# autonomousvision/sdfstudio

Measured on NVIDIA H100. Metric: rays/sec at 4096 rays x 128 samples, higher is better.
Workload: dtype bf16x3 (fp32 accumulate)

## Files before the change

include/sdfb200_debug.h:

```cpp
#ifndef SDFB200_DEBUG_H_
#define SDFB200_DEBUG_H_
#include "sdfb200.h"
#ifdef __cplusplus
extern "C" {
#endif

int sdfb200_debug_tc_gemm(const float* A, const float* W, int32_t K, int32_t N, int32_t mode_ts, int32_t planes, float* D,
                          void* scratch, void* stream);

int sdfb200_debug_tc_linear(int32_t planes, int32_t epi, const float* X, int32_t ldx, const float* W, const float* bias, float* Y,
                            int32_t ldy, int64_t M, int32_t Np, int32_t Kp, const float* aux, int32_t ldaux, int32_t aux_cols,
                            void* scratch, void* stream);

int sdfb200_debug_tc_timing(long long* host_out_512);

#ifdef __cplusplus
}
#endif
#endif
```

sdfstudio_b200/csrc/field_tc.h:

```cpp
#pragma once
#include "field_plan.h"

namespace sdfb200 {


constexpr int kEpiWarps = 8;
constexpr int kEpiThreads = kEpiWarps * 32;
constexpr int kTcThreads = kEpiThreads + 128;
constexpr int kEncThreads = 96;
constexpr int kEncItems0 = 288, kEncItems1 = 256, kEncItems2 = 224;
static_assert(kEncItems0 + kEncItems1 + kEncItems2 == 768, "the encoder warps' items cover the tile");
__host__ __device__ constexpr int enc_item_begin(int w) { return w == 0 ? 0 : w == 1 ? kEncItems0 : w == 2 ? kEncItems0 + kEncItems1 : 768; }
constexpr int kConsumerRegs = 216;
constexpr int kProducerRegs = 72;
static_assert(2 * (kConsumerRegs - 168) <= 168 - kProducerRegs, "setmaxnreg.inc would wait for registers nobody frees");
constexpr int kStages = 5;
constexpr int kKB = 16;
constexpr int kMaxGridDim = 32;
constexpr int kMaxPe = 60;
constexpr int kPeRows = 64;
constexpr int kInK = 96;
constexpr float kHalfPiF = 1.5707963267948966f;
constexpr uint32_t kAPlane = 32 * 2048;
constexpr uint32_t kImgPlane = (kInK / 8) * 128 * 16;
__host__ __device__ constexpr uint32_t tc_stage_bytes(int planes) { return (uint32_t)planes * 256 * kKB * 2; }

enum { PRM_B_G0 = 0, PRM_B_G1, PRM_W_G2 , PRM_B_C0, PRM_B_C1, PRM_W_C2 , kPrmRows = PRM_W_C2 + 3 };
enum { HS_SDF = 0, HS_GRAD , HS_RGB = HS_GRAD + 3 , kHsRows = HS_RGB + 3 };

struct TcSmem { size_t a, ring, prm, hs, coldesc, hx, bytes; };
__host__ __device__ constexpr TcSmem tc_smem(int planes) {
  TcSmem s{};
  s.ring = s.a + (size_t)planes * kAPlane;
  s.prm = s.ring + (size_t)kStages * tc_stage_bytes(planes);
  s.hs = s.prm + kPrmRows * 256 * 4;
  s.coldesc = s.hs + 2 * kHsRows * 128 * 4;
  s.hx = s.coldesc + 96 * 16;
  s.bytes = s.hx + 128 * 8;
  return s;
}
constexpr size_t kSmemPerBlock = 232448;
constexpr size_t kStaticSmem = 1024;
static_assert(tc_smem(2).bytes + kStaticSmem <= kSmemPerBlock, "shared memory of k_field_tc at two planes");

constexpr size_t kFragWords = 64 * 256;
struct TcScratch { size_t sig, h2, slots, slot_bytes, geo, cs, jpe, jg, bytes; };
__host__ __device__ constexpr TcScratch tc_scratch(int planes) {
  TcScratch s{};
  s.h2 = s.sig + kFragWords * 4;
  s.slots = s.h2 + (size_t)planes * kFragWords * 4;
  s.cs = s.geo + (size_t)planes * kImgPlane;
  s.jpe = s.cs + (size_t)planes * kImgPlane;
  s.jg = s.jpe + (size_t)kPeRows * 128 * 4;
  s.slot_bytes = s.jg + (size_t)kMaxGridDim * 3 * 128 * 4;
  s.bytes = s.slots + 2 * s.slot_bytes;
  return s;
}
__host__ __device__ constexpr size_t kScratchPerCta(int planes) { return tc_scratch(planes).bytes; }

__host__ __device__ constexpr int tc_layer_np(int L) { return L == L_B0 ? 128 : 256; }
__host__ __device__ constexpr int tc_layer_k(int L) { return L == L_G0 || L == L_C0MISC ? kInK : 256; }
__host__ __device__ constexpr int tc_layer_kblk(int L) { return kKB * 256 / tc_layer_np(L); }
__host__ __device__ constexpr int tc_layer_nkb(int L) { return tc_layer_k(L) / tc_layer_kblk(L); }
constexpr bool tc_blocks_fill_stages() {
  for (int L = 0; L < L_COUNT; ++L)
    if (tc_layer_np(L) * tc_layer_kblk(L) != 256 * kKB || tc_layer_kblk(L) % 16 != 0 || tc_layer_k(L) % tc_layer_kblk(L) != 0) return false;
  return true;
}
static_assert(tc_blocks_fill_stages(), "every streamed weight block must be one full ring stage of whole K steps");

struct TcLayer {
  unsigned long long w_off;
};

struct TcArgs {
  sdfb200_grid_t grid;
  TcLayer layer[L_COUNT];
  int use_grid, pe_degree, use_pe, contraction, pe_dim, grid_dim, app_dim, use_n_dot_v;
  int mode;
  int n_samples, has_bins, n_tiles;
  long long n_points;
  float rgb_padding, cos_anneal;
  const float *origins, *directions, *bins, *appearance, *variance, *beta, *beta_min;
  const void* table;
  const char* blob;
  unsigned long long b_g0, b_g1, b_g2, w_g2, b_c0, b_c1, w_c2, b_c2;
  char* scratch;
  sdfb200_field_out_t out;
  int render;
  sdfb200_field_render_t rnd;
};

int launch_field_tc_p2_torch(const TcArgs& a, int grid, size_t smem, cudaStream_t st);
int launch_field_tc_p2_tcnn(const TcArgs& a, int grid, size_t smem, cudaStream_t st);
int launch_field_tc_p1_torch(const TcArgs& a, int grid, size_t smem, cudaStream_t st);
int launch_field_tc_p1_tcnn(const TcArgs& a, int grid, size_t smem, cudaStream_t st);

}
```

sdfstudio_b200/csrc/field_tc_kernel.cuh:

```cuda
#pragma once
#include "field_tc.h"
#include "grid.cuh"
#include "tc_common.cuh"

namespace sdfb200 {
using namespace tc;

__device__ __forceinline__ void named_sync(int id, int n) { asm volatile("bar.sync %0, %1;" ::"r"(id), "r"(n) : "memory"); }
constexpr int kEncBar = 3;

struct PointGeom { float px, py, pz, dx, dy, dz, delta, t0, t1; long long ray; };
__device__ __forceinline__ PointGeom point_geom(const TcArgs& a, long long p) {
  PointGeom g;
  g.dx = g.dy = g.dz = 0.f; g.delta = 0.f; g.t0 = g.t1 = 0.f;
  g.ray = a.has_bins ? p / a.n_samples : p;
  if (a.has_bins) {
    const int smp = (int)(p - g.ray * a.n_samples);
    const float t0 = __ldg(a.bins + g.ray * (a.n_samples + 1) + smp);
    g.t0 = t0;
    g.t1 = __ldg(a.bins + g.ray * (a.n_samples + 1) + smp + 1);
    g.delta = __fsub_rn(g.t1, t0);
    g.dx = __ldg(a.directions + g.ray * 3); g.dy = __ldg(a.directions + g.ray * 3 + 1); g.dz = __ldg(a.directions + g.ray * 3 + 2);
    g.px = __fadd_rn(__ldg(a.origins + g.ray * 3 + 0), __fmul_rn(g.dx, t0));
    g.py = __fadd_rn(__ldg(a.origins + g.ray * 3 + 1), __fmul_rn(g.dy, t0));
    g.pz = __fadd_rn(__ldg(a.origins + g.ray * 3 + 2), __fmul_rn(g.dz, t0));
  } else {
    g.px = __ldg(a.origins + p * 3); g.py = __ldg(a.origins + p * 3 + 1); g.pz = __ldg(a.origins + p * 3 + 2);
    if (a.directions) { g.dx = __ldg(a.directions + p * 3); g.dy = __ldg(a.directions + p * 3 + 1); g.dz = __ldg(a.directions + p * 3 + 2); }
  }
  if (a.contraction != SDFB200_CONTRACT_NONE) {
    const float mag = a.contraction == SDFB200_CONTRACT_LINF
                          ? fmaxf(fabsf(g.px), fmaxf(fabsf(g.py), fabsf(g.pz)))
                          : sqrtf(__fadd_rn(__fadd_rn(__fmul_rn(g.px, g.px), __fmul_rn(g.py, g.py)), __fmul_rn(g.pz, g.pz)));
    if (mag >= 1.f) {
      const float k = __fsub_rn(2.f, __fdiv_rn(1.f, mag));
      g.px = __fmul_rn(k, __fdiv_rn(g.px, mag)); g.py = __fmul_rn(k, __fdiv_rn(g.py, mag)); g.pz = __fmul_rn(k, __fdiv_rn(g.pz, mag));
    }
  }
  return g;
}

static __device__ __forceinline__ void sincos_call(float x, float* s, float* c) { sincosf(x, s, c); }
static __device__ __forceinline__ float sin_call(float x) { return sinf(x); }

template <int P, int LAYOUT>
__device__ __forceinline__ void encode_tile_grid(const TcArgs& a, int tile, int row, int grp, uint8_t* img, uint32_t plane, float* Jg,
                                                 uint64_t pol_table) {
  const long long p_raw = (long long)tile * 128 + row;
  const long long p = p_raw < a.n_points ? p_raw : a.n_points - 1;
  const PointGeom g = point_geom(a, p);
  const float x01 = (g.px + 2.0f) * 0.25f, y01 = (g.py + 2.0f) * 0.25f, z01 = (g.pz + 2.0f) * 0.25f;
#pragma unroll 1
  for (int l = 4 * grp; l < 4 * grp + 4; ++l) {
    float o[2] = {0.f, 0.f};
    float dj[2][3] = {{0.f, 0.f, 0.f}, {0.f, 0.f, 0.f}};
    if (a.use_grid && l < a.grid.n_levels && l < a.grid.active_levels) {
      LevelCtx c;
      float tv[8][2];
      level_prepare<LAYOUT>(a.grid, l, x01, y01, z01, c);
      if (a.grid.table_dtype == SDFB200_DT_F16) level_fetch<__half, 2, true>(a.table, c, tv, pol_table);
      else level_fetch<float, 2, true>(a.table, c, tv, pol_table);
      level_finish<2, LAYOUT>(a.grid, c, tv, o, dj);
    }
    store_a<P>(img, plane, row, 2 * l, o[0]);
    store_a<P>(img, plane, row, 2 * l + 1, o[1]);
    if (a.mode != 0 && l < a.grid.n_levels) {
#pragma unroll
      for (int f = 0; f < 2; ++f) {
        const int cg = l * 2 + f;
        Jg[(cg * 3 + 0) * 128 + row] = 0.25f * dj[f][0];
        Jg[(cg * 3 + 1) * 128 + row] = 0.25f * dj[f][1];
        Jg[(cg * 3 + 2) * 128 + row] = 0.25f * dj[f][2];
      }
    }
  }
}

template <int P>
__device__ __forceinline__ void encode_tile_pe(const TcArgs& a, int tile, int row, uint8_t* img, uint32_t plane, float* Jpe) {
  const long long p_raw = (long long)tile * 128 + row;
  const long long p = p_raw < a.n_points ? p_raw : a.n_points - 1;
  const PointGeom g = point_geom(a, p);
  if (p_raw < a.n_points) {
    if (a.out.points_norm) a.out.points_norm[p] = sqrtf(__fadd_rn(__fadd_rn(__fmul_rn(g.px, g.px), __fmul_rn(g.py, g.py)), __fmul_rn(g.pz, g.pz)));
    if (a.out.points) { a.out.points[p * 3] = g.px; a.out.points[p * 3 + 1] = g.py; a.out.points[p * 3 + 2] = g.pz; }
  }
  const int deg = a.pe_degree, half = 3 * deg;
  const float pc[3] = {g.px, g.py, g.pz};
  const uint4 z4 = make_uint4(0u, 0u, 0u, 0u);
#pragma unroll 1
  for (int ch = 4; ch < kInK / 8; ++ch) store_a_chunk<P>(img, plane, row, ch, z4, z4);
#pragma unroll 1
  for (int i = 0; i < a.pe_dim; ++i) {
    const int ia = i >= half ? i - half : i;
    const int b = ia / deg, k = ia - b * deg;
    const float fr = (float)(1 << k);
    const float xb = b == 0 ? pc[0] : (b == 1 ? pc[1] : pc[2]);
    const float arg = i >= half ? xb * fr + kHalfPiF : xb * fr;
    float sv, cv;
    sincos_call(arg, &sv, &cv);
    store_a<P>(img, plane, row, 32 + i, a.use_pe ? sv : 0.f);
    if (a.mode != 0) Jpe[i * 128 + row] = a.use_pe ? fr * cv : 0.f;
  }
  store_a<P>(img, plane, row, 32 + a.pe_dim + 0, pc[0]);
  store_a<P>(img, plane, row, 32 + a.pe_dim + 1, pc[1]);
  store_a<P>(img, plane, row, 32 + a.pe_dim + 2, pc[2]);
}

template <int P>
__device__ __forceinline__ void colour_static_tile(const TcArgs& a, int tile, int row, uint8_t* img, uint32_t plane) {
  const long long p_raw = (long long)tile * 128 + row;
  const long long p = p_raw < a.n_points ? p_raw : a.n_points - 1;
  const PointGeom g = point_geom(a, p);
  const uint4 z4 = make_uint4(0u, 0u, 0u, 0u);
#pragma unroll 1
  for (int ch = 1; ch < kInK / 8; ++ch) store_a_chunk<P>(img, plane, row, ch, z4, z4);
  store_a<P>(img, plane, row, 8 + 0, g.px); store_a<P>(img, plane, row, 8 + 1, g.py); store_a<P>(img, plane, row, 8 + 2, g.pz);
#pragma unroll 1
  for (int i = 0; i < 12; ++i) {
    const int b = i >> 2;
    const float db = b == 0 ? g.dx : (b == 1 ? g.dy : g.dz);
    const float arg = db * (float)(1 << (i & 3));
    store_a<P>(img, plane, row, 8 + 3 + i, sin_call(arg));
    store_a<P>(img, plane, row, 8 + 15 + i, sin_call(arg + kHalfPiF));
  }
  store_a<P>(img, plane, row, 8 + 27, g.dx); store_a<P>(img, plane, row, 8 + 28, g.dy); store_a<P>(img, plane, row, 8 + 29, g.dz);
  if (a.appearance != nullptr) {
#pragma unroll 1
    for (int j = 0; j < a.app_dim; ++j) store_a<P>(img, plane, row, 8 + 30 + j, __ldg(a.appearance + g.ray * a.app_dim + j));
  }
}

template <int P>
struct Slot {
  uint8_t* base;
  __device__ __forceinline__ Slot(char* slots, uint32_t s) : base(reinterpret_cast<uint8_t*>(slots) + s * tc_scratch(P).slot_bytes) {}
  __device__ __forceinline__ uint8_t* geo() const { return base + tc_scratch(P).geo; }
  __device__ __forceinline__ uint8_t* cs() const { return base + tc_scratch(P).cs; }
  __device__ __forceinline__ float* jpe() const { return reinterpret_cast<float*>(base + tc_scratch(P).jpe); }
  __device__ __forceinline__ float* jg() const { return reinterpret_cast<float*>(base + tc_scratch(P).jg); }
};

#ifdef SDFB200_TC_TIMING
__device__ long long g_tc_timing[16 * 32];
#define TC_PUT(tno, k, v)                                                                                            \
  do {                                                                                                               \
    if (blockIdx.x == 0 && (tno) >= 0 && (tno) < 16) g_tc_timing[(tno) * 32 + (k)] = (v);                            \
  } while (0)
#else
#define TC_PUT(tno, k, v) do { (void)(v); } while (0)
#endif
#define TC_STAMP(k) do { if (tid == 0) TC_PUT(tile_no, k, TC_CLOCK()); } while (0)

struct TcBars {
  Handoff<kStages> ring;
  Handoff<2> enc;
  Handoff<1> a;
  Handoff<2> hs;
};

template <int P>
__device__ __forceinline__ void produce_all(const TcArgs& a, int nlayers, uint8_t* abuf, uint8_t* ring, char* slots, TcBars& b) {
  uint32_t j = 0;
  int tile_no = 0;
  for (int tile = blockIdx.x; tile < a.n_tiles; tile += gridDim.x, ++tile_no) {
    long long waited = 0;
    b.a.wait_empty(tile_no);
    b.enc.wait_full(tile_no);
    const uint8_t* geo = Slot<P>(slots, b.enc.slot(tile_no)).geo();
    mbar_arrive_expect_tx(b.a.full_bar(tile_no), (uint32_t)P * kImgPlane);
#pragma unroll
    for (int pl = 0; pl < P; ++pl) bulk_g2s(abuf + pl * kAPlane, geo + pl * kImgPlane, kImgPlane, b.a.full_bar(tile_no));
    for (int L = 0; L < nlayers; ++L) {
      for (int kb = 0; kb < tc_layer_nkb(L); ++kb, ++j)
        ring_fill(b.ring, ring, j, reinterpret_cast<const uint8_t*>(a.blob) + a.layer[L].w_off, kb, tc_stage_bytes(P), &waited);
    }
    TC_PUT(tile_no, 10, waited);
  }
}

template <int P, int L>
__device__ __forceinline__ void layer_mma(float (&acc)[4][32], bool zero, uint32_t a_base, const uint8_t* ring, Handoff<kStages>& rb, uint32_t& it,
                                          int lane, long long& waited) {
  constexpr int N = tc_layer_np(L);
  constexpr int KSTEPS = tc_layer_kblk(L) / 16;
  constexpr uint32_t lbo_b = N * 16, plane_b = N * KSTEPS * 16 * 2;
  float (&d)[N / 2] = *reinterpret_cast<float (*)[N / 2]>(&acc[0][0]);
  if (zero) {
#pragma unroll
    for (int i = 0; i < N / 2; ++i) d[i] = 0.f;
  }
#pragma unroll 1
  for (int kb = 0; kb < tc_layer_nkb(L); ++kb, ++it) {
    rb.wait_full(it, &waited);
    const uint32_t wbase = smem_u32(ring + (size_t)rb.slot(it) * tc_stage_bytes(P));
    wg_fence_acc(d);
    wg_arrive();
#pragma unroll
    for (int j = 0; j < KSTEPS; ++j) {
      const int kstep = kb * KSTEPS + j;
      wgmma_kstep_wide_ss<P, N>(d, a_desc(a_base, kstep), a_desc(a_base + kAPlane, kstep), wbase + j * 2 * lbo_b, plane_b, lbo_b);
    }
    wg_commit();
    wg_wait<0>();
    wg_fence_acc(d);
    __syncwarp();
    if (lane == 0) rb.arrive_empty(it);
  }
}

struct TileCtx {
  const TcArgs& a;
  int tid, t, wg, wrow0;
  int r0, cq;
  uint8_t* abuf;
  const float (*prm)[256];
  float (*hs)[128];
  const float4* coldesc;
  float sdf_bias;
  uint32_t* sig_s;
  uint32_t* gf_s;
  char* slots;
  __device__ __forceinline__ int unit(int c, int i) const { return (c * 16 + (i >> 1)) * kEpiThreads + tid; }
};

__device__ __forceinline__ uint32_t unorm16x2_encode(float s0, float s1) {
  const float f0 = __fadd_rn(__fmul_rn(s0, 65535.0f), 12582912.0f), f1 = __fadd_rn(__fmul_rn(s1, 65535.0f), 12582912.0f);
  return __byte_perm(__float_as_uint(f0), __float_as_uint(f1), 0x5410);
}
__device__ __forceinline__ float unorm16_lo(uint32_t w) { return __fsub_rn(__uint_as_float(__byte_perm(w, 0x4B00u, 0x5410)), 8388608.0f) * (1.0f / 65535.0f); }
__device__ __forceinline__ float unorm16_hi(uint32_t w) { return __fsub_rn(__uint_as_float(__byte_perm(w, 0x4B00u, 0x5432)), 8388608.0f) * (1.0f / 65535.0f); }

__device__ __forceinline__ void acc_shift(float (&acc)[4][32]) {
#pragma unroll
  for (int c = 0; c < 3; ++c) {
#pragma unroll
    for (int i = 0; i < 32; ++i) acc[c][i] = acc[c + 1][i];
  }
}

template <int N>
__device__ __forceinline__ void load_prm_block(const float* prow, int cq, int c, int j0, float2 (&v)[N]) {
#pragma unroll
  for (int j = 0; j < N; ++j) v[j] = *reinterpret_cast<const float2*>(prow + frag_col(cq, c, 4 * (j0 + j)));
}

template <int P>
__device__ __forceinline__ void epi_e0(const TileCtx& x, float (&acc)[4][32]) {
  const float* p_bg0 = x.prm[PRM_B_G0];
#pragma unroll 1
  for (int c = 0; c < 4; ++c, acc_shift(acc)) {
    float2 bias[8];
    load_prm_block(p_bg0, x.cq, c, 0, bias);
#pragma unroll
    for (int i = 0; i < 32; i += 2) {
      const int col = frag_col(x.cq, c, i), row = frag_row(x.r0, i);
      const float2 b2 = bias[i >> 2];
      float h0, h1, s0, s1;
      softplus100_fast(acc[0][i] + b2.x, h0, s0);
      softplus100_fast(acc[0][i + 1] + b2.y, h1, s1);
      store_a_pair<P>(x.abuf, kAPlane, row, col, h0, h1);
      if (x.a.mode != 0) x.sig_s[x.unit(c, i)] = unorm16x2_encode(s0, s1);
    }
  }
}

template <int P>
__device__ __forceinline__ void epi_e1(const TileCtx& x, int tile, float (&acc)[4][32]) {
  const TcArgs& a = x.a;
  const float* p_bg1 = x.prm[PRM_B_G1];
  const float* p_wg2 = x.prm[PRM_W_G2];
  float sp0 = 0.f, sp1 = 0.f;
#pragma unroll 1
  for (int c = 0; c < 4; ++c, acc_shift(acc)) {
    float2 bias[2], wrow[2];
#pragma unroll
    for (int i = 0; i < 32; i += 2) {
      if (i % 8 == 0) { load_prm_block(p_bg1, x.cq, c, i >> 2, bias); load_prm_block(p_wg2, x.cq, c, i >> 2, wrow); }
      const int col = frag_col(x.cq, c, i), row = frag_row(x.r0, i);
      const float2 b2 = bias[(i >> 2) & 1];
      const float2 w2 = wrow[(i >> 2) & 1];
      float h0, h1, s0, s1;
      softplus100_fast(acc[0][i] + b2.x, h0, s0);
      softplus100_fast(acc[0][i + 1] + b2.y, h1, s1);
      float& sp = frag_half(i) ? sp1 : sp0;
      sp = fmaf(w2.x, h0, sp);
      sp = fmaf(w2.y, h1, sp);
      if (a.mode != 0) {
        uint32_t hi, lo;
        split2(h0, h1, hi, lo);
        const int u = x.unit(c, i);
        x.gf_s[u] = hi;
        if (P > 1) x.gf_s[kFragWords + u] = lo;
        store_a_pair<P>(x.abuf, kAPlane, row, col, w2.x * s0, w2.y * s1);
      }
    }
  }
  sp0 = quad_sum(sp0);
  sp1 = quad_sum(sp1);
  if ((x.t & 3) < 2) {
    const int h = x.t & 1, row = x.r0 + 8 * h;
    const float sdf = (h ? sp1 : sp0) + x.sdf_bias;
    const long long p = (long long)tile * 128 + row;
    if (p < a.n_points && a.out.sdf) a.out.sdf[p] = sdf;
    if (a.mode != 0) x.hs[HS_SDF][row] = sdf;
  }
}

template <int P>
__device__ __forceinline__ void epi_eb1(const TileCtx& x, float (&acc)[4][32]) {
  uint32_t sw[16], sw_next[16];
#pragma unroll
  for (int k = 0; k < 16; ++k) sw[k] = x.sig_s[x.unit(0, 2 * k)];
#pragma unroll 1
  for (int c = 0; c < 4; ++c, acc_shift(acc)) {
    if (c < 3) {
#pragma unroll
      for (int k = 0; k < 16; ++k) sw_next[k] = x.sig_s[x.unit(c + 1, 2 * k)];
    }
#pragma unroll
    for (int i = 0; i < 32; i += 2) {
      const int col = frag_col(x.cq, c, i), row = frag_row(x.r0, i);
      const uint32_t w = sw[i >> 1];
      store_a_pair<P>(x.abuf, kAPlane, row, col, acc[0][i] * unorm16_lo(w), acc[0][i + 1] * unorm16_hi(w));
    }
    if (c < 3) {
#pragma unroll
      for (int k = 0; k < 16; ++k) sw[k] = sw_next[k];
    }
  }
}

__device__ __forceinline__ float4 col_desc(const TcArgs& a, int ip) {
  const int deg = a.pe_degree, half = 3 * deg;
  int jrow = -1, ax = -1;
  if (ip < a.pe_dim) {
    const int ia = ip >= half ? ip - half : ip;
    ax = ia < deg ? 0 : (ia < 2 * deg ? 1 : 2);
    jrow = ip * 128;
  } else if (ip - a.pe_dim < 3) {
    ax = ip - a.pe_dim;
  }
  return make_float4(__int_as_float(jrow), ax == 0 ? 1.f : 0.f, ax == 1 ? 1.f : 0.f, ax == 2 ? 1.f : 0.f);
}

template <int P>
__device__ __forceinline__ void epi_eb0(const TileCtx& x, int tile, const Slot<P>& s, const float (&acc)[4][32]) {
  const TcArgs& a = x.a;
  const float* Jpe = s.jpe();
  const float* Jg = s.jg();
  constexpr int kUnits = 11 * 64 * P, kPer = (kUnits + 127) / 128;
  uint4 v[kPer];
#pragma unroll
  for (int j = 0; j < kPer; ++j) {
    const int k = x.t + 128 * j, pl = k / (11 * 64), ch = 1 + (k - pl * 11 * 64) / 64, row = x.wrow0 + (k & 63);
    if (k < kUnits) v[j] = *reinterpret_cast<const uint4*>(s.cs() + pl * kImgPlane + ch * kAChunk + row * 16);
  }
  float g0x = 0.f, g0y = 0.f, g0z = 0.f, g1x = 0.f, g1y = 0.f, g1z = 0.f;
#pragma unroll
  for (int c = 0; c < 2; ++c) {
#pragma unroll
    for (int i = 0; i < 32; ++i) {
      const int col = frag_col(x.cq, c, i), row = frag_row(x.r0, i);
      const bool h = frag_half(i);
      float& gx = h ? g1x : g0x;
      float& gy = h ? g1y : g0y;
      float& gz = h ? g1z : g0z;
      const float g = acc[c][i];
      if (c == 0 && i < 16) {
        const bool live = col < a.grid_dim;
        const float* j = Jg + col * 3 * 128 + row;
        const float jx = live ? j[0] : 0.f, jy = live ? j[128] : 0.f, jz = live ? j[256] : 0.f;
        gx = fmaf(g, jx, gx); gy = fmaf(g, jy, gy); gz = fmaf(g, jz, gz);
      } else {
        const float4 d = x.coldesc[col - 32];
        const int jrow = __float_as_int(d.x);
        const float tv = __fmul_rn(g, jrow >= 0 ? Jpe[jrow + row] : 1.f);
        gx = fmaf(tv, d.y, gx); gy = fmaf(tv, d.z, gy); gz = fmaf(tv, d.w, gz);
      }
    }
  }
  g0x = quad_sum(g0x); g0y = quad_sum(g0y); g0z = quad_sum(g0z);
  g1x = quad_sum(g1x); g1y = quad_sum(g1y); g1z = quad_sum(g1z);
  if ((x.t & 3) < 2) {
    const int h = x.t & 1, row = x.r0 + 8 * h;
    const long long p_raw = (long long)tile * 128 + row;
    const PointGeom pg = point_geom(a, p_raw < a.n_points ? p_raw : a.n_points - 1);
    const float grx = h ? g1x : g0x, gry = h ? g1y : g0y, grz = h ? g1z : g0z;
    const float3 n = normalize_eps(grx, gry, grz);
    const float c0v[8] = {grx, gry, grz, a.use_n_dot_v ? n.x * pg.dx + n.y * pg.dy + n.z * pg.dz : 0.f, 0.f, 0.f, 0.f, 0.f};
    store_a_chunk<P>(x.abuf, kAPlane, row, 0, c0v);
    x.hs[HS_GRAD][row] = grx; x.hs[HS_GRAD + 1][row] = gry; x.hs[HS_GRAD + 2][row] = grz;
  }
#pragma unroll
  for (int j = 0; j < kPer; ++j) {
    const int k = x.t + 128 * j, pl = k / (11 * 64), ch = 1 + (k - pl * 11 * 64) / 64, row = x.wrow0 + (k & 63);
    if (k < kUnits) *reinterpret_cast<uint4*>(x.abuf + pl * kAPlane + ch * kAChunk + row * 16) = v[j];
  }
}

template <int P>
__device__ __forceinline__ void reload_h2(const TileCtx& x) {
#pragma unroll 1
  for (int c = 0; c < 4; ++c) {
#pragma unroll
    for (int i = 0; i < 32; i += 2) {
      const int col = frag_col(x.cq, c, i), row = frag_row(x.r0, i);
      const int u = x.unit(c, i);
      store_a_pair<P>(x.abuf, kAPlane, row, col, x.gf_s[u], x.gf_s[kFragWords + u]);
    }
  }
}

template <int P>
__device__ __forceinline__ void epi_ec0(const TileCtx& x, float (&acc)[4][32]) {
  const float* p_bc0 = x.prm[PRM_B_C0];
#pragma unroll 1
  for (int c = 0; c < 4; ++c, acc_shift(acc)) {
    float2 bias[8];
    load_prm_block(p_bc0, x.cq, c, 0, bias);
#pragma unroll
    for (int i = 0; i < 32; i += 2) {
      const int col = frag_col(x.cq, c, i), row = frag_row(x.r0, i);
      const float2 b2 = bias[i >> 2];
      store_a_pair<P>(x.abuf, kAPlane, row, col, fmaxf(acc[0][i] + b2.x, 0.f), fmaxf(acc[0][i + 1] + b2.y, 0.f));
    }
  }
}

__device__ __forceinline__ void epi_ec1(const TileCtx& x, float (&acc)[4][32]) {
  const float* p_bc1 = x.prm[PRM_B_C1];
  const float (*p_wc2)[256] = x.prm + PRM_W_C2;
  float r0r = 0.f, r0g = 0.f, r0b = 0.f, r1r = 0.f, r1g = 0.f, r1b = 0.f;
#pragma unroll 1
  for (int c = 0; c < 4; ++c, acc_shift(acc)) {
#pragma unroll
    for (int i = 0; i < 32; ++i) {
      const int col = frag_col(x.cq, c, i);
      const bool h = frag_half(i);
      float& rr = h ? r1r : r0r;
      float& rg = h ? r1g : r0g;
      float& rb = h ? r1b : r0b;
      const float v = fmaxf(acc[0][i] + p_bc1[col], 0.f);
      rr = fmaf(p_wc2[0][col], v, rr);
      rg = fmaf(p_wc2[1][col], v, rg);
      rb = fmaf(p_wc2[2][col], v, rb);
    }
  }
  r0r = quad_sum(r0r); r0g = quad_sum(r0g); r0b = quad_sum(r0b);
  r1r = quad_sum(r1r); r1g = quad_sum(r1g); r1b = quad_sum(r1b);
  if ((x.t & 3) < 2) {
    const int h = x.t & 1, row = x.r0 + 8 * h;
    x.hs[HS_RGB][row] = h ? r1r : r0r; x.hs[HS_RGB + 1][row] = h ? r1g : r0g; x.hs[HS_RGB + 2][row] = h ? r1b : r0b;
  }
}

struct HeadsXfer { double wtot[2][4]; float csum[2][4][8]; };
static_assert(sizeof(TcBars) + sizeof(HeadsXfer) <= kStaticSmem, "static shared memory of k_field_tc (kStaticSmem)");
enum { HR_ALPHA = HS_SDF , HR_NORMAL = HS_GRAD , HR_RGB = HS_RGB  };
struct RayEnd { int q; double tot; float last[3]; };
struct HeadsClock { long long rows, scan, sums; };

__device__ __forceinline__ float sample_mid(const TcArgs& a, long long p) {
// ... 134 lines not shown
#pragma unroll
      for (int k = 0; k < 8; ++k) s[k] += csum[w2][k];
    }
    finish_ray(ray, s[0], {s[1], s[2], s[3]}, {s[4], s[5], s[6]}, s[7], a.rnd.bg_mode, a.rnd.bg, end.last, a.rnd.clamp01, a.rnd.out.rgb,
               a.rnd.out.accumulation, a.rnd.out.normal, a.rnd.out.depth);
    const bool dens = a.rnd.from_density != 0;
    if (a.rnd.bg_transmittance) a.rnd.bg_transmittance[ray] = dens ? expf(-(float)end.tot) : (float)end.tot;
  }
  clk.sums += TC_CLOCK() - tc0;
}

__device__ __forceinline__ void heads_of(const TcArgs& a, int tile, int tile_no, int et, TcBars& b, float (*hs)[128], double* hx, HeadsXfer& xf,
                                         float& dmin, float& dmax) {
  const int ew = et >> 5, lane = et & 31;
  long long waited = 0, bar_waited = 0;
  b.hs.wait_full(tile_no, &waited);
  const long long t0 = TC_CLOCK();
  float (*h)[128] = hs + b.hs.slot(tile_no) * kHsRows;
  double* wtot = xf.wtot[tile_no & 1];
  float (*csum)[8] = xf.csum[tile_no & 1];
  HeadsClock clk{0, 0, 0};
#pragma unroll 1
  for (int q = ew; q < 4; q += kEncThreads / 32) heads_rows(a, h, hx, wtot, tile, q, lane, dmin, dmax, clk);
  if (a.render && a.n_samples > 32) {
    long long c = TC_CLOCK();
    named_sync(kEncBar, kEncThreads);
    bar_waited += TC_CLOCK() - c;
    RayEnd end{-1, 0.0, {0.f, 0.f, 0.f}};
#pragma unroll 1
    for (int q = ew; q < 4; q += kEncThreads / 32) composite_chunk(a, h, hx, wtot, csum, tile, q, lane, end, clk);
    c = TC_CLOCK();
    named_sync(kEncBar, kEncThreads);
    bar_waited += TC_CLOCK() - c;
    finish_rays(a, csum, tile, lane, end, clk);
  }
  b.hs.arrive_empty(tile_no);
  if (lane == 0) TC_PUT(tile_no, ew == 0 ? 14 : 25 + ew, TC_CLOCK() - t0);
  if (et == 0) { TC_PUT(tile_no, 17, waited); TC_PUT(tile_no, 28, clk.rows); TC_PUT(tile_no, 29, clk.scan); TC_PUT(tile_no, 30, clk.sums); TC_PUT(tile_no, 31, bar_waited); }
}

template <int P, int LAYOUT>
__device__ __forceinline__ void encode_all(const TcArgs& a, int et, char* slots, TcBars& b, uint64_t pol_table, float (*hs)[128], double* hx,
                                           HeadsXfer& xf) {
  const bool heads = a.mode != 0;
  const int ew = et >> 5, lane = et & 31;
  const int i_begin = heads ? enc_item_begin(ew) + lane : et, i_end = heads ? enc_item_begin(ew + 1) : 640, i_step = heads ? 32 : kEncThreads;
  float dmin = INFINITY, dmax = -INFINITY;
  int tile_no = 0;
  for (int tile = blockIdx.x; tile < a.n_tiles; tile += gridDim.x, ++tile_no) {
    long long waited = 0;
    b.enc.wait_empty(tile_no, &waited);
    const long long t0 = TC_CLOCK();
    const Slot<P> s(slots, b.enc.slot(tile_no));
#pragma unroll 1
    for (int i = i_begin; i < i_end; i += i_step) {
      const int row = i & 127;
      if (i < 512) encode_tile_grid<P, LAYOUT>(a, tile, row, i >> 7, s.geo(), kImgPlane, s.jg(), pol_table);
      else if (i < 640) encode_tile_pe<P>(a, tile, row, s.geo(), kImgPlane, s.jpe());
      else colour_static_tile<P>(a, tile, row, s.cs(), kImgPlane);
    }
    fence_async_global();
    b.enc.arrive_full(tile_no);
    if (et == 0) { TC_PUT(tile_no, 12, TC_CLOCK() - t0); TC_PUT(tile_no, 13, waited); }
    else if (lane == 0) TC_PUT(tile_no, 23 + ew, TC_CLOCK() - t0);
    if (heads && tile_no > 0) heads_of(a, tile - (int)gridDim.x, tile_no - 1, et, b, hs, hx, xf, dmin, dmax);
  }
  if (heads && tile_no > 0) heads_of(a, blockIdx.x + (tile_no - 1) * (int)gridDim.x, tile_no - 1, et, b, hs, hx, xf, dmin, dmax);
  if (heads && a.render && a.rnd.out.steps_minmax) {
#pragma unroll
    for (int d = 1; d < 32; d <<= 1) {
      dmin = fminf(dmin, __shfl_xor_sync(0xffffffffu, dmin, d));
      dmax = fmaxf(dmax, __shfl_xor_sync(0xffffffffu, dmax, d));
    }
    if (lane == 0 && dmin <= dmax) { atomic_min_float(a.rnd.out.steps_minmax, dmin); atomic_max_float(a.rnd.out.steps_minmax + 1, dmax); }
  }
}

template <int P, int LAYOUT>
__global__ void __launch_bounds__(kTcThreads, 1) k_field_tc(const __grid_constant__ TcArgs a) {
  extern __shared__ __align__(1024) uint8_t smem[];
  constexpr TcSmem sm = tc_smem(P);
  constexpr TcScratch scr = tc_scratch(P);
  uint8_t* abuf = smem + sm.a;
  uint8_t* ring = smem + sm.ring;
  float (*prm)[256] = reinterpret_cast<float (*)[256]>(smem + sm.prm);
  float (*hs)[128] = reinterpret_cast<float (*)[128]>(smem + sm.hs);
  float4* coldesc = reinterpret_cast<float4*>(smem + sm.coldesc);
  double* hx = reinterpret_cast<double*>(smem + sm.hx);
  __shared__ TcBars bars;
  __shared__ HeadsXfer hxf;

  const int tid = threadIdx.x, warp = tid >> 5, lane = tid & 31;
  const int nlayers = a.mode == 0 ? 2 : L_COUNT;
  char* cta_scr = a.scratch + (size_t)blockIdx.x * scr.bytes;
  char* slots = cta_scr + scr.slots;
  if (tid == 0) {
    bars.ring.init(1, kEpiWarps);
    bars.enc.init(kEncThreads, kEpiThreads);
    bars.hs.init(kEpiThreads, kEncThreads);
    bars.a.init(1, 2);
    fence_barrier_init();
  }
  {
    const char* blob = a.blob;
    const float* src[kPrmRows] = {reinterpret_cast<const float*>(blob + a.b_g0), reinterpret_cast<const float*>(blob + a.b_g1),
                                  reinterpret_cast<const float*>(blob + a.w_g2), reinterpret_cast<const float*>(blob + a.b_c0),
                                  reinterpret_cast<const float*>(blob + a.b_c1), reinterpret_cast<const float*>(blob + a.w_c2),
                                  reinterpret_cast<const float*>(blob + a.w_c2) + 256, reinterpret_cast<const float*>(blob + a.w_c2) + 512};
    for (int i = tid; i < kPrmRows * 256; i += kTcThreads) prm[i >> 8][i & 255] = src[i >> 8][i & 255];
    if (tid < 96) coldesc[tid] = col_desc(a, tid);
  }
  __syncthreads();

  if (tid >= kEpiThreads) {
    setmaxnreg_dec<kProducerRegs>();
    if (tid == kEpiThreads) produce_all<P>(a, nlayers, abuf, ring, slots, bars);
    else if (tid >= kTcThreads - kEncThreads) encode_all<P, LAYOUT>(a, tid - (kTcThreads - kEncThreads), slots, bars, l2_policy_evict_last(), hs, hx, hxf);
    return;
  }
  setmaxnreg_inc<kConsumerRegs>();

  const int wg = warp >> 2, t = tid & 127;
  const int wrow0 = wg * 64;
  const int wg_bar = 1 + wg;
  const uint32_t a_base = smem_u32(abuf) + wrow0 * 16;
  const float sdf_bias = __ldg(reinterpret_cast<const float*>(a.blob + a.b_g2));
  TileCtx x{a, tid, t, wg, wrow0, frag_row0(wrow0, t), frag_cq(t), abuf, prm, hs, coldesc, sdf_bias,
            reinterpret_cast<uint32_t*>(cta_scr + scr.sig), reinterpret_cast<uint32_t*>(cta_scr + scr.h2), slots};
  uint32_t it = 0;
  long long waited = 0;
  float acc[4][32];
#define SYNC_A()                \
  do {                          \
    fence_async_smem();         \
    named_sync(wg_bar, 128);    \
  } while (0)
#define LAYER(L, zero)                                                                                 \
  do {                                                                                                 \
    layer_mma<P, L>(acc, zero, a_base, ring, bars.ring, it, lane, waited);                             \
    named_sync(wg_bar, 128);   \
    TC_STAMP(1 + (L));                                                                                 \
  } while (0)

  int tile_no = -1;
  for (int tile = blockIdx.x; tile < a.n_tiles; tile += gridDim.x) {
    ++tile_no;
    TC_STAMP(0);
    waited = 0;
    const Slot<P> s(slots, bars.enc.slot(tile_no));
    x.hs = hs + bars.hs.slot(tile_no) * kHsRows;
    bars.a.wait_full(tile_no);
    if (a.mode == 0) bars.enc.arrive_empty(tile_no);
    TC_STAMP(8);
    LAYER(L_G0, true);
    epi_e0<P>(x, acc);
    TC_STAMP(18);
    SYNC_A();
    LAYER(L_G1, true);
    if (a.mode == 0) {
      if (t == 0) bars.a.arrive_empty(tile_no);
      epi_e1<P>(x, tile, acc);
      continue;
    }
    {
      long long hs_waited = 0;
      bars.hs.wait_empty(tile_no, &hs_waited);
      if (tid == 0) TC_PUT(tile_no, 16, hs_waited);
    }
    epi_e1<P>(x, tile, acc);
    TC_STAMP(19);
    SYNC_A();
    LAYER(L_B1, true);
    epi_eb1<P>(x, acc);
    TC_STAMP(20);
    SYNC_A();
    LAYER(L_B0, true);
    bars.enc.wait_full(tile_no);
    epi_eb0<P>(x, tile, s, acc);
    bars.enc.arrive_empty(tile_no);
    TC_STAMP(21);
    SYNC_A();
    LAYER(L_C0MISC, true);
    reload_h2<P>(x);
    TC_STAMP(22);
    SYNC_A();
    LAYER(L_C0H, false);
    epi_ec0<P>(x, acc);
    TC_STAMP(23);
    SYNC_A();
    LAYER(L_C1, true);
    if (t == 0) bars.a.arrive_empty(tile_no);
    epi_ec1(x, acc);
    bars.hs.arrive_full(tile_no);
    TC_STAMP(15);
    if (tid == 0) TC_PUT(tile_no, 9, waited);
  }
#undef SYNC_A
#undef LAYER
}

template <int P, int LAYOUT>
static int launch_field_tc(const TcArgs& a, int grid, size_t smem, cudaStream_t st) {
  SDFB_CUDA(cudaFuncSetAttribute(k_field_tc<P, LAYOUT>, cudaFuncAttributeMaxDynamicSharedMemorySize, (int)smem));
  k_field_tc<P, LAYOUT><<<grid, kTcThreads, smem, st>>>(a);
  SDFB_LAUNCHED("k_field_tc");
  return 0;
}

}
```

sdfstudio_b200/csrc/field_tc_p2_torch.cu:

```cuda
#include "field_tc_kernel.cuh"

namespace sdfb200 {
int launch_field_tc_p2_torch(const TcArgs& a, int grid, size_t smem, cudaStream_t st) { return launch_field_tc<2, SDFB200_GRID_TORCH>(a, grid, smem, st); }
}

#ifdef SDFB200_TC_TIMING
extern "C" int sdfb200_debug_tc_timing(long long* host_out_512) {
  SDFB_CUDA(cudaMemcpyFromSymbol(host_out_512, sdfb200::g_tc_timing, sizeof(long long) * 512));
  return 0;
}
#endif
```

sdfstudio_b200/csrc/grid.cuh:

```cuda
#pragma once
#include "common.cuh"

namespace sdfb200 {

constexpr uint32_t kPrimeY = 2654435761u;
constexpr uint32_t kPrimeZ = 805459861u;

__device__ __forceinline__ uint64_t l2_policy_evict_last() {
  uint64_t p;
  asm volatile("createpolicy.fractional.L2::evict_last.b64 %0, 1.0;" : "=l"(p));
  return p;
}

template <typename T, int F, bool HINT = false>
__device__ __forceinline__ void load_row(const void* table, uint64_t row, float (&v)[F], uint64_t pol = 0) {
  const T* p = reinterpret_cast<const T*>(table) + row * F;
  if constexpr (HINT) {
    static_assert(F == 2, "hinted loads are only used by the F=2 fused kernel");
    if constexpr (sizeof(T) == 4) {
      asm volatile("ld.global.nc.L2::cache_hint.v2.f32 {%0, %1}, [%2], %3;" : "=f"(v[0]), "=f"(v[1]) : "l"(p), "l"(pol));
    } else {
      uint32_t raw;
      asm volatile("ld.global.nc.L2::cache_hint.b32 %0, [%1], %2;" : "=r"(raw) : "l"(p), "l"(pol));
      const float2 t = __half22float2(*reinterpret_cast<const __half2*>(&raw));
// ... 47 lines not shown
  uint32_t idx[8];
  uint64_t base;
  float w[3], dw[3], d2w[3], s;
};

template <int LAYOUT = -1>
__device__ __forceinline__ void level_prepare(const sdfb200_grid_t& g, int l, float x, float y, float z, LevelCtx& c) {
  if constexpr (LAYOUT < 0) {
    if (g.layout == SDFB200_GRID_TORCH) level_prepare<SDFB200_GRID_TORCH>(g, l, x, y, z, c);
    else level_prepare<SDFB200_GRID_TCNN>(g, l, x, y, z, c);
    return;
  }
  constexpr bool torch = LAYOUT == SDFB200_GRID_TORCH;
  const float s = g.scale[l];
  const float xs[3] = {x, y, z};
  uint32_t lo[3], hi[3];
  c.s = s;
  c.base = g.offset[l];
#pragma unroll
  for (int d = 0; d < 3; ++d) {
    const float p = torch ? __fmul_rn(xs[d], s) : fmaf(xs[d], s, 0.5f);
    const float fl = floorf(p);
    lo[d] = (uint32_t)(int)fl;
    hi[d] = torch ? (uint32_t)(int)ceilf(p) : lo[d] + 1u;
    const float t = __fsub_rn(p, fl);
    if (g.smoothstep) {
      c.w[d] = __fmul_rn(__fmul_rn(t, t), __fsub_rn(3.0f, __fmul_rn(2.0f, t)));
      c.dw[d] = 6.f * t * (1.f - t);
      c.d2w[d] = (6.f - 12.f * t) * s * s;
    } else {
      c.w[d] = t; c.dw[d] = 1.f; c.d2w[d] = 0.f;
    }
  }
  const uint32_t mask = (1u << g.log2_hashmap_size) - 1u;
#pragma unroll
  for (int k = 0; k < 8; ++k) {
    const uint32_t ix = (k & 1) ? hi[0] : lo[0], iy = (k & 2) ? hi[1] : lo[1], iz = (k & 4) ? hi[2] : lo[2];
    const uint32_t h = ix ^ (iy * kPrimeY) ^ (iz * kPrimeZ);
    if (torch) {
      c.idx[k] = h & mask;
    } else {
      const uint32_t res = g.resolution[l];
      c.idx[k] = (g.hashed[l] ? h : ix + iy * res + iz * res * res) % g.size[l];
    }
  }
}

template <typename T, int F, bool HINT = false>
__device__ __forceinline__ void level_fetch(const void* table, const LevelCtx& c, float (&v)[8][F], uint64_t pol = 0) {
#pragma unroll
  for (int k = 0; k < 8; ++k) load_row<T, F, HINT>(table, c.base + c.idx[k], v[k], pol);
}

template <int F, int LAYOUT = -1>
__device__ __forceinline__ void level_finish(const sdfb200_grid_t& g, const LevelCtx& c, const float (&v)[8][F], float (&out)[F], float (&dout)[F][3]) {
  if (torch_layout<LAYOUT>(g)) {
    const float(&f0)[F] = v[7], (&f1)[F] = v[5], (&f2)[F] = v[4], (&f3)[F] = v[6], (&f4)[F] = v[3], (&f5)[F] = v[1], (&f6)[F] = v[0], (&f7)[F] = v[2];
    const float ox = c.w[0], oy = c.w[1], oz = c.w[2];
    const float nx = __fsub_rn(1.f, ox), ny = __fsub_rn(1.f, oy), nz = __fsub_rn(1.f, oz);
#pragma unroll
    for (int f = 0; f < F; ++f) {
      const float f03 = __fadd_rn(__fmul_rn(f0[f], ox), __fmul_rn(f3[f], nx));
      const float f12 = __fadd_rn(__fmul_rn(f1[f], ox), __fmul_rn(f2[f], nx));
      const float f56 = __fadd_rn(__fmul_rn(f5[f], ox), __fmul_rn(f6[f], nx));
      const float f47 = __fadd_rn(__fmul_rn(f4[f], ox), __fmul_rn(f7[f], nx));
      const float f0312 = __fadd_rn(__fmul_rn(f03, oy), __fmul_rn(f12, ny));
      const float f4756 = __fadd_rn(__fmul_rn(f47, oy), __fmul_rn(f56, ny));
      out[f] = __fadd_rn(__fmul_rn(f0312, oz), __fmul_rn(f4756, nz));
      const float gx = ((f0[f] - f3[f]) * oy + (f1[f] - f2[f]) * ny) * oz + ((f4[f] - f7[f]) * oy + (f5[f] - f6[f]) * ny) * nz;
      const float gy = (f03 - f12) * oz + (f47 - f56) * nz;
      const float gz = f0312 - f4756;
      dout[f][0] = gx * c.dw[0] * c.s; dout[f][1] = gy * c.dw[1] * c.s; dout[f][2] = gz * c.dw[2] * c.s;
    }
  } else {
#pragma unroll
    for (int f = 0; f < F; ++f) { out[f] = 0.f; dout[f][0] = dout[f][1] = dout[f][2] = 0.f; }
#pragma unroll
    for (int k = 0; k < 8; ++k) {
      const float wx = (k & 1) ? c.w[0] : 1.f - c.w[0], wy = (k & 2) ? c.w[1] : 1.f - c.w[1], wz = (k & 4) ? c.w[2] : 1.f - c.w[2];
      const float wt = wx * wy * wz;
#pragma unroll
      for (int f = 0; f < F; ++f) {
        out[f] = fmaf(wt, v[k][f], out[f]);
        dout[f][0] += ((k & 1) ? 1.f : -1.f) * wy * wz * v[k][f];
        dout[f][1] += ((k & 2) ? 1.f : -1.f) * wx * wz * v[k][f];
        dout[f][2] += ((k & 4) ? 1.f : -1.f) * wx * wy * v[k][f];
      }
    }
#pragma unroll
    for (int f = 0; f < F; ++f) { dout[f][0] *= c.dw[0] * c.s; dout[f][1] *= c.dw[1] * c.s; dout[f][2] *= c.dw[2] * c.s; }
  }
}

template <typename T, int F>
__device__ __forceinline__ void encode_level(const sdfb200_grid_t& g, const void* table, int l, float x, float y, float z,
                                             float (&out)[F], float (&dout)[F][3]) {
  LevelCtx c;
  float v[8][F];
  level_prepare(g, l, x, y, z, c);
  level_fetch<T, F>(table, c, v);
  level_finish<F>(g, c, v, out, dout);
}

__device__ __forceinline__ void corner_weights(const LevelCtx& c, float (&w)[8]) {
#pragma unroll
  for (int k = 0; k < 8; ++k)
// ... 5 lines not shown
```

Baseline: 1.393 million.

## Stage colour inputs and h2 via bulk async copies, prefetch hash rows, share direction encoding

The h2 activations are now stored directly in A-operand image layout in scratch. They and the static colour chunks are brought back into the A buffer with bulk global-to-shared copies tracked by new mbarriers, replacing the register-staged copy in epi_eb0 and the reload_h2 loop. The C0H layer reorders its K steps so it can start on the early-copied chunks and waits on the late-copy barrier only midway. The grid encoder also issues L2 prefetches for all corner rows of a point's levels before fetching them, and colour encoding computes the 24 sin terms once per warp when all lanes share a ray, broadcasting them by shuffle. Per-kind encoder timing counters are added under the timing build flag. The changes add barrier complexity and extra prefetch instructions.

Result: faster. 1.446 million (median of 6 runs) (+3.8%).

```diff
diff --git a/include/sdfb200_debug.h b/include/sdfb200_debug.h
--- a/include/sdfb200_debug.h
+++ b/include/sdfb200_debug.h
@@ -12,7 +12,7 @@
                             int32_t ldy, int64_t M, int32_t Np, int32_t Kp, const float* aux, int32_t ldaux, int32_t aux_cols,
                             void* scratch, void* stream);
 
-int sdfb200_debug_tc_timing(long long* host_out_512);
+int sdfb200_debug_tc_timing(long long* host_out_768);
 
 #ifdef __cplusplus
 }
diff --git a/sdfstudio_b200/csrc/field_tc.h b/sdfstudio_b200/csrc/field_tc.h
--- a/sdfstudio_b200/csrc/field_tc.h
+++ b/sdfstudio_b200/csrc/field_tc.h
@@ -10,6 +10,7 @@
 constexpr int kEncThreads = 96;
 constexpr int kEncItems0 = 288, kEncItems1 = 256, kEncItems2 = 224;
 static_assert(kEncItems0 + kEncItems1 + kEncItems2 == 768, "the encoder warps' items cover the tile");
+static_assert(kEncItems0 % 32 == 0 && kEncItems1 % 32 == 0, "a warp stages whole 32-row batches (colour_static_tile shuffles across them)");
 __host__ __device__ constexpr int enc_item_begin(int w) { return w == 0 ? 0 : w == 1 ? kEncItems0 : w == 2 ? kEncItems0 + kEncItems1 : 768; }
 constexpr int kConsumerRegs = 216;
 constexpr int kProducerRegs = 72;
@@ -48,7 +49,7 @@
 __host__ __device__ constexpr TcScratch tc_scratch(int planes) {
   TcScratch s{};
   s.h2 = s.sig + kFragWords * 4;
-  s.slots = s.h2 + (size_t)planes * kFragWords * 4;
+  s.slots = s.h2 + (size_t)planes * kAPlane;
   s.cs = s.geo + (size_t)planes * kImgPlane;
   s.jpe = s.cs + (size_t)planes * kImgPlane;
   s.jg = s.jpe + (size_t)kPeRows * 128 * 4;
diff --git a/sdfstudio_b200/csrc/field_tc_kernel.cuh b/sdfstudio_b200/csrc/field_tc_kernel.cuh
--- a/sdfstudio_b200/csrc/field_tc_kernel.cuh
+++ b/sdfstudio_b200/csrc/field_tc_kernel.cuh
@@ -50,11 +50,21 @@
   const long long p = p_raw < a.n_points ? p_raw : a.n_points - 1;
   const PointGeom g = point_geom(a, p);
   const float x01 = (g.px + 2.0f) * 0.25f, y01 = (g.py + 2.0f) * 0.25f, z01 = (g.pz + 2.0f) * 0.25f;
+  const int l_end = min(4 * grp + 4, min(a.grid.n_levels, a.grid.active_levels));
+  if (a.use_grid && a.mode != 0) {
+#pragma unroll 1
+    for (int l = 4 * grp; l < l_end; ++l) {
+      LevelCtx c;
+      level_prepare<LAYOUT>(a.grid, l, x01, y01, z01, c);
+      if (a.grid.table_dtype == SDFB200_DT_F16) level_prefetch_l2<__half, 2>(a.table, c);
+      else level_prefetch_l2<float, 2>(a.table, c);
+    }
+  }
 #pragma unroll 1
   for (int l = 4 * grp; l < 4 * grp + 4; ++l) {
     float o[2] = {0.f, 0.f};
     float dj[2][3] = {{0.f, 0.f, 0.f}, {0.f, 0.f, 0.f}};
-    if (a.use_grid && l < a.grid.n_levels && l < a.grid.active_levels) {
+    if (a.use_grid && l < l_end) {
       LevelCtx c;
       float tv[8][2];
       level_prepare<LAYOUT>(a.grid, l, x01, y01, z01, c);
@@ -107,23 +117,27 @@
   store_a<P>(img, plane, row, 32 + a.pe_dim + 2, pc[2]);
 }
 
+__device__ __forceinline__ float dir_enc(const PointGeom& g, int k) {
+  const int i = k < 12 ? k : k - 12, b = i >> 2;
+  const float db = b == 0 ? g.dx : (b == 1 ? g.dy : g.dz);
+  const float arg = db * (float)(1 << (i & 3));
+  return sin_call(k < 12 ? arg : arg + kHalfPiF);
+}
+
 template <int P>
 __device__ __forceinline__ void colour_static_tile(const TcArgs& a, int tile, int row, uint8_t* img, uint32_t plane) {
   const long long p_raw = (long long)tile * 128 + row;
   const long long p = p_raw < a.n_points ? p_raw : a.n_points - 1;
   const PointGeom g = point_geom(a, p);
+  const bool one_ray = __match_any_sync(0xffffffffu, g.ray) == 0xffffffffu;
+  const int lane = row & 31;
+  const float own = one_ray && lane < 24 ? dir_enc(g, lane) : 0.f;
   const uint4 z4 = make_uint4(0u, 0u, 0u, 0u);
 #pragma unroll 1
   for (int ch = 1; ch < kInK / 8; ++ch) store_a_chunk<P>(img, plane, row, ch, z4, z4);
   store_a<P>(img, plane, row, 8 + 0, g.px); store_a<P>(img, plane, row, 8 + 1, g.py); store_a<P>(img, plane, row, 8 + 2, g.pz);
 #pragma unroll 1
-  for (int i = 0; i < 12; ++i) {
-    const int b = i >> 2;
-    const float db = b == 0 ? g.dx : (b == 1 ? g.dy : g.dz);
-    const float arg = db * (float)(1 << (i & 3));
-    store_a<P>(img, plane, row, 8 + 3 + i, sin_call(arg));
-    store_a<P>(img, plane, row, 8 + 15 + i, sin_call(arg + kHalfPiF));
-  }
+  for (int k = 0; k < 24; ++k) store_a<P>(img, plane, row, 8 + 3 + k, one_ray ? __shfl_sync(0xffffffffu, own, k) : dir_enc(g, k));
   store_a<P>(img, plane, row, 8 + 27, g.dx); store_a<P>(img, plane, row, 8 + 28, g.dy); store_a<P>(img, plane, row, 8 + 29, g.dz);
   if (a.appearance != nullptr) {
 #pragma unroll 1
@@ -142,10 +156,10 @@
 };
 
 #ifdef SDFB200_TC_TIMING
-__device__ long long g_tc_timing[16 * 32];
+__device__ long long g_tc_timing[16 * 48];
 #define TC_PUT(tno, k, v)                                                                                            \
   do {                                                                                                               \
-    if (blockIdx.x == 0 && (tno) >= 0 && (tno) < 16) g_tc_timing[(tno) * 32 + (k)] = (v);                            \
+    if (blockIdx.x == 0 && (tno) >= 0 && (tno) < 16) g_tc_timing[(tno) * 48 + (k)] = (v);                            \
   } while (0)
 #else
 #define TC_PUT(tno, k, v) do { (void)(v); } while (0)
@@ -157,6 +171,7 @@
   Handoff<2> enc;
   Handoff<1> a;
   Handoff<2> hs;
+  uint64_t cop[2][2];
 };
 
 template <int P>
@@ -179,9 +194,10 @@
   }
 }
 
+constexpr int kH2Early = 32 - kInK / 8;
 template <int P, int L>
 __device__ __forceinline__ void layer_mma(float (&acc)[4][32], bool zero, uint32_t a_base, const uint8_t* ring, Handoff<kStages>& rb, uint32_t& it,
-                                          int lane, long long& waited) {
+                                          int lane, long long& waited, uint64_t* h2_late, uint32_t h2_parity) {
   constexpr int N = tc_layer_np(L);
   constexpr int KSTEPS = tc_layer_kblk(L) / 16;
   constexpr uint32_t lbo_b = N * 16, plane_b = N * KSTEPS * 16 * 2;
@@ -192,6 +208,7 @@
   }
 #pragma unroll 1
   for (int kb = 0; kb < tc_layer_nkb(L); ++kb, ++it) {
+    if (L == L_C0H && kb * KSTEPS == kH2Early / 2) mbar_wait(h2_late, h2_parity);
     rb.wait_full(it, &waited);
     const uint32_t wbase = smem_u32(ring + (size_t)rb.slot(it) * tc_stage_bytes(P));
     wg_fence_acc(d);
@@ -199,7 +216,8 @@
 #pragma unroll
     for (int j = 0; j < KSTEPS; ++j) {
       const int kstep = kb * KSTEPS + j;
-      wgmma_kstep_wide_ss<P, N>(d, a_desc(a_base, kstep), a_desc(a_base + kAPlane, kstep), wbase + j * 2 * lbo_b, plane_b, lbo_b);
+      const int ka = L == L_C0H ? (kstep + kInK / 16) % 16 : kstep;
+      wgmma_kstep_wide_ss<P, N>(d, a_desc(a_base, ka), a_desc(a_base + kAPlane, ka), wbase + j * 2 * lbo_b, plane_b, lbo_b);
     }
     wg_commit();
     wg_wait<0>();
@@ -219,7 +237,7 @@
   const float4* coldesc;
   float sdf_bias;
   uint32_t* sig_s;
-  uint32_t* gf_s;
+  uint8_t* h2img;
   char* slots;
   __device__ __forceinline__ int unit(int c, int i) const { return (c * 16 + (i >> 1)) * kEpiThreads + tid; }
 };
@@ -287,15 +305,12 @@
       sp = fmaf(w2.x, h0, sp);
       sp = fmaf(w2.y, h1, sp);
       if (a.mode != 0) {
-        uint32_t hi, lo;
-        split2(h0, h1, hi, lo);
-        const int u = x.unit(c, i);
-        x.gf_s[u] = hi;
-        if (P > 1) x.gf_s[kFragWords + u] = lo;
+        store_a_pair<P>(x.h2img, kAPlane, row, col, h0, h1);
         store_a_pair<P>(x.abuf, kAPlane, row, col, w2.x * s0, w2.y * s1);
       }
     }
   }
+  if (a.mode != 0) fence_async_global();
   sp0 = quad_sum(sp0);
   sp1 = quad_sum(sp1);
   if ((x.t & 3) < 2) {
@@ -345,17 +360,32 @@
 }
 
 template <int P>
+__device__ __forceinline__ void copy_chunks(uint8_t* abuf, int a_chunk, const uint8_t* src, uint32_t src_plane, int src_chunk, int n, int wrow0,
+                                            uint64_t* bar, int lane) {
+  for (int k = lane; k < P * n; k += 32) {
+    const int pl = k / n, c = k - pl * n;
+    bulk_g2s(abuf + pl * kAPlane + (a_chunk + c) * kAChunk + wrow0 * 16, src + pl * src_plane + (src_chunk + c) * kAChunk + wrow0 * 16, 64 * 16, bar);
+  }
+}
+template <int P>
+__device__ __forceinline__ void colour_copy(const TileCtx& x, bool early, const uint8_t* cs, uint64_t* bar) {
+  constexpr int kMisc = kInK / 8;
+  const int lane = x.t & 31;
+  if (lane == 0) mbar_arrive_expect_tx(bar, (uint32_t)P * (early ? (kMisc - 1) + kH2Early : 32 - kH2Early) * 64 * 16);
+  __syncwarp();
+  if (early) {
+    copy_chunks<P>(x.abuf, 1, cs, kImgPlane, 1, kMisc - 1, x.wrow0, bar, lane);
+    copy_chunks<P>(x.abuf, kMisc, x.h2img, kAPlane, 0, kH2Early, x.wrow0, bar, lane);
+  } else {
+    copy_chunks<P>(x.abuf, 0, x.h2img, kAPlane, kH2Early, 32 - kH2Early, x.wrow0, bar, lane);
+  }
+}
+
+template <int P>
 __device__ __forceinline__ void epi_eb0(const TileCtx& x, int tile, const Slot<P>& s, const float (&acc)[4][32]) {
   const TcArgs& a = x.a;
   const float* Jpe = s.jpe();
   const float* Jg = s.jg();
-  constexpr int kUnits = 11 * 64 * P, kPer = (kUnits + 127) / 128;
-  uint4 v[kPer];
-#pragma unroll
-  for (int j = 0; j < kPer; ++j) {
-    const int k = x.t + 128 * j, pl = k / (11 * 64), ch = 1 + (k - pl * 11 * 64) / 64, row = x.wrow0 + (k & 63);
-    if (k < kUnits) v[j] = *reinterpret_cast<const uint4*>(s.cs() + pl * kImgPlane + ch * kAChunk + row * 16);
-  }
   float g0x = 0.f, g0y = 0.f, g0z = 0.f, g1x = 0.f, g1y = 0.f, g1z = 0.f;
 #pragma unroll
   for (int c = 0; c < 2; ++c) {
@@ -391,24 +421,6 @@
     const float c0v[8] = {grx, gry, grz, a.use_n_dot_v ? n.x * pg.dx + n.y * pg.dy + n.z * pg.dz : 0.f, 0.f, 0.f, 0.f, 0.f};
     store_a_chunk<P>(x.abuf, kAPlane, row, 0, c0v);
     x.hs[HS_GRAD][row] = grx; x.hs[HS_GRAD + 1][row] = gry; x.hs[HS_GRAD + 2][row] = grz;
-  }
-#pragma unroll
-  for (int j = 0; j < kPer; ++j) {
-    const int k = x.t + 128 * j, pl = k / (11 * 64), ch = 1 + (k - pl * 11 * 64) / 64, row = x.wrow0 + (k & 63);
-    if (k < kUnits) *reinterpret_cast<uint4*>(x.abuf + pl * kAPlane + ch * kAChunk + row * 16) = v[j];
-  }
-}
-
-template <int P>
-__device__ __forceinline__ void reload_h2(const TileCtx& x) {
-#pragma unroll 1
-  for (int c = 0; c < 4; ++c) {
-#pragma unroll
-    for (int i = 0; i < 32; i += 2) {
-      const int col = frag_col(x.cq, c, i), row = frag_row(x.r0, i);
-      const int u = x.unit(c, i);
-      store_a_pair<P>(x.abuf, kAPlane, row, col, x.gf_s[u], x.gf_s[kFragWords + u]);
-    }
   }
 }
 
@@ -649,17 +661,20 @@
     b.enc.wait_empty(tile_no, &waited);
     const long long t0 = TC_CLOCK();
     const Slot<P> s(slots, b.enc.slot(tile_no));
+    long long kind_grid = 0, kind_pe = 0, kind_cs = 0;
 #pragma unroll 1
     for (int i = i_begin; i < i_end; i += i_step) {
       const int row = i & 127;
-      if (i < 512) encode_tile_grid<P, LAYOUT>(a, tile, row, i >> 7, s.geo(), kImgPlane, s.jg(), pol_table);
-      else if (i < 640) encode_tile_pe<P>(a, tile, row, s.geo(), kImgPlane, s.jpe());
-      else colour_static_tile<P>(a, tile, row, s.cs(), kImgPlane);
+      const long long c0 = TC_CLOCK();
+      if (i < 512) { encode_tile_grid<P, LAYOUT>(a, tile, row, i >> 7, s.geo(), kImgPlane, s.jg(), pol_table); kind_grid += TC_CLOCK() - c0; }
+      else if (i < 640) { encode_tile_pe<P>(a, tile, row, s.geo(), kImgPlane, s.jpe()); kind_pe += TC_CLOCK() - c0; }
+      else { colour_static_tile<P>(a, tile, row, s.cs(), kImgPlane); kind_cs += TC_CLOCK() - c0; }
     }
     fence_async_global();
     b.enc.arrive_full(tile_no);
     if (et == 0) { TC_PUT(tile_no, 12, TC_CLOCK() - t0); TC_PUT(tile_no, 13, waited); }
     else if (lane == 0) TC_PUT(tile_no, 23 + ew, TC_CLOCK() - t0);
+    if (lane == 0) { TC_PUT(tile_no, 32 + 3 * ew, kind_grid); TC_PUT(tile_no, 33 + 3 * ew, kind_pe); TC_PUT(tile_no, 34 + 3 * ew, kind_cs); }
     if (heads && tile_no > 0) heads_of(a, tile - (int)gridDim.x, tile_no - 1, et, b, hs, hx, xf, dmin, dmax);
   }
   if (heads && tile_no > 0) heads_of(a, blockIdx.x + (tile_no - 1) * (int)gridDim.x, tile_no - 1, et, b, hs, hx, xf, dmin, dmax);
@@ -696,6 +711,7 @@
     bars.enc.init(kEncThreads, kEpiThreads);
     bars.hs.init(kEpiThreads, kEncThreads);
     bars.a.init(1, 2);
+    for (int w = 0; w < 2; ++w) { mbar_init(&bars.cop[w][0], 1); mbar_init(&bars.cop[w][1], 1); }
     fence_barrier_init();
   }
   {
@@ -723,7 +739,7 @@
   const uint32_t a_base = smem_u32(abuf) + wrow0 * 16;
   const float sdf_bias = __ldg(reinterpret_cast<const float*>(a.blob + a.b_g2));
   TileCtx x{a, tid, t, wg, wrow0, frag_row0(wrow0, t), frag_cq(t), abuf, prm, hs, coldesc, sdf_bias,
-            reinterpret_cast<uint32_t*>(cta_scr + scr.sig), reinterpret_cast<uint32_t*>(cta_scr + scr.h2), slots};
+            reinterpret_cast<uint32_t*>(cta_scr + scr.sig), reinterpret_cast<uint8_t*>(cta_scr + scr.h2), slots};
   uint32_t it = 0;
   long long waited = 0;
   float acc[4][32];
@@ -734,7 +750,7 @@
   } while (0)
 #define LAYER(L, zero)                                                                                 \
   do {                                                                                                 \
-    layer_mma<P, L>(acc, zero, a_base, ring, bars.ring, it, lane, waited);                             \
+    layer_mma<P, L>(acc, zero, a_base, ring, bars.ring, it, lane, waited, &bars.cop[wg][1], tile_no & 1); \
     named_sync(wg_bar, 128);   \
     TC_STAMP(1 + (L));                                                                                 \
   } while (0)
@@ -773,14 +789,15 @@
     SYNC_A();
     LAYER(L_B0, true);
     bars.enc.wait_full(tile_no);
+    if (t < 32) colour_copy<P>(x, true, s.cs(), &bars.cop[wg][0]);
     epi_eb0<P>(x, tile, s, acc);
+    mbar_wait(&bars.cop[wg][0], tile_no & 1);
     bars.enc.arrive_empty(tile_no);
     TC_STAMP(21);
     SYNC_A();
     LAYER(L_C0MISC, true);
-    reload_h2<P>(x);
+    if (t < 32) colour_copy<P>(x, false, nullptr, &bars.cop[wg][1]);
     TC_STAMP(22);
-    SYNC_A();
     LAYER(L_C0H, false);
     epi_ec0<P>(x, acc);
     TC_STAMP(23);
diff --git a/sdfstudio_b200/csrc/field_tc_p2_torch.cu b/sdfstudio_b200/csrc/field_tc_p2_torch.cu
--- a/sdfstudio_b200/csrc/field_tc_p2_torch.cu
+++ b/sdfstudio_b200/csrc/field_tc_p2_torch.cu
@@ -5,8 +5,8 @@
 }
 
 #ifdef SDFB200_TC_TIMING
-extern "C" int sdfb200_debug_tc_timing(long long* host_out_512) {
-  SDFB_CUDA(cudaMemcpyFromSymbol(host_out_512, sdfb200::g_tc_timing, sizeof(long long) * 512));
+extern "C" int sdfb200_debug_tc_timing(long long* host_out_768) {
+  SDFB_CUDA(cudaMemcpyFromSymbol(host_out_768, sdfb200::g_tc_timing, sizeof(sdfb200::g_tc_timing)));
   return 0;
 }
 #endif
diff --git a/sdfstudio_b200/csrc/grid.cuh b/sdfstudio_b200/csrc/grid.cuh
--- a/sdfstudio_b200/csrc/grid.cuh
+++ b/sdfstudio_b200/csrc/grid.cuh
@@ -123,6 +123,13 @@
   for (int k = 0; k < 8; ++k) load_row<T, F, HINT>(table, c.base + c.idx[k], v[k], pol);
 }
 
+template <typename T, int F>
+__device__ __forceinline__ void level_prefetch_l2(const void* table, const LevelCtx& c) {
+#pragma unroll
+  for (int k = 0; k < 8; ++k)
+    asm volatile("prefetch.global.L2::evict_last [%0];" ::"l"(reinterpret_cast<const T*>(table) + (c.base + c.idx[k]) * F));
+}
+
 template <int F, int LAYOUT = -1>
 __device__ __forceinline__ void level_finish(const sdfb200_grid_t& g, const LevelCtx& c, const float (&v)[8][F], float (&out)[F], float (&dout)[F][3]) {
   if (torch_layout<LAYOUT>(g)) {
```
